# zju3dv/clean-pvnet

Hardware: NVIDIA B200
Metric: ransac_vote_throughput (higher is better)
Workload: dtype f32

## Files before the change

clean_pvnet_b200/csrc/api.cu:

```cuda
#include <cmath>
#include <cstdarg>
#include <cstdio>
#include <cstring>
#include <new>
#include <vector>
#include "kernels.h"

using namespace pvb;

namespace {

thread_local char g_err[512] = "";

int fail(int code, const char *fmt, ...)
{
    va_list ap;
    va_start(ap, fmt);
    vsnprintf(g_err, sizeof(g_err), fmt, ap);
    va_end(ap);
    return code;
}

int cuda_fail(cudaError_t e, const char *what)
{
// ... 55 lines not shown
    if ((long long)d->K * ((d->hn + 511) / 512) > 65535) return fail(PVB_ERR_INVALID, "K*ceil(hn/512) must be <= 65535");
    if (d->mask_dtype < PVB_MASK_U8 || d->mask_dtype > PVB_MASK_F64) return fail(PVB_ERR_INVALID, "bad mask_dtype %d", d->mask_dtype);
    if (d->select_mode != PVB_SELECT_BYTE && d->select_mode != PVB_SELECT_EQ1)
        return fail(PVB_ERR_INVALID, "bad select_mode %d", d->select_mode);
    return PVB_OK;
}

int make_layout(const pvb_desc *d, pvb_layout *L)
{
    const int rc = check_desc(d);
    if (rc) return rc;
    const size_t B = (size_t)d->B, K = (size_t)d->K, hn = (size_t)d->hn;
    const int nwords = (int)(((long long)d->H * d->W + 31) / 32);
    const int nblocks = (nwords + 127) / 128;
    const int cap = default_capacity(d);
    const int splits = refit_splits_for(cap);
    size_t off = 0;
    auto take = [&](size_t bytes) { const size_t o = off; off = align_up(off + bytes); return o; };
    L->status = take(4 * sizeof(int));
    L->fgsum = take(B * sizeof(unsigned long long));
    L->nz = take(B * sizeof(int));
    L->tn = take(B * sizeof(int));
    L->state = take(B * sizeof(int));
    L->refit_ticket = take(B * K * sizeof(int));
    L->ticket = take(B * sizeof(int));
    L->blocktot = take(B * nblocks * sizeof(int));
    L->bits = take(B * nwords * sizeof(uint32_t));
    L->xy = take(B * cap * sizeof(float2));
    L->dirs = take(B * K * cap * sizeof(float2));
    L->hyp = take(B * K * hn * sizeof(float2));
    L->counts = take(B * K * hn * sizeof(int));
    L->win = take(B * K * sizeof(float2));
    L->refit_partial = take(B * K * splits * 5 * sizeof(double));
    L->total = off;
    L->nwords = nwords;
    L->nblocks = nblocks;
    L->capacity = cap;
    L->refit_splits = splits;
    return PVB_OK;
}

struct Plan {
    pvb_layout L;
    SelectArgs s;
    VoteArgs v;
    float2 *win;
    RefitScratch refit;
};

int make_plan(const pvb_desc *d, const void *mask, const float *vertex, const int32_t *idxs,
              const float *selection, void *ws, size_t ws_bytes, uint32_t tag_idx, uint32_t tag_sel, Plan *P)
{
    int rc = make_layout(d, &P->L);
    if (rc) return rc;
    if (!mask || !vertex) return fail(PVB_ERR_INVALID, "mask/vertex is NULL");
    if (!ws || ws_bytes < P->L.total) return fail(PVB_ERR_WORKSPACE, "workspace too small: need %zu bytes, got %zu", P->L.total, ws_bytes);
    if (reinterpret_cast<uintptr_t>(ws) & 255u) return fail(PVB_ERR_WORKSPACE, "workspace must be 256-byte aligned");
    char *w = static_cast<char *>(ws);
    const pvb_layout &L = P->L;
    SelectArgs &s = P->s;
    s.mask = mask; s.mask_dtype = d->mask_dtype; s.select_mode = d->select_mode;
    s.msb = d->mask_stride[0]; s.msy = d->mask_stride[1]; s.msx = d->mask_stride[2];
    s.vertex = vertex;
    for (int i = 0; i < 5; ++i) s.vs[i] = d->vertex_stride[i];
    s.selection = selection;
    s.B = d->B; s.H = d->H; s.W = d->W; s.K = d->K; s.nwords = L.nwords; s.nblocks = L.nblocks; s.cap = L.capacity;
    s.min_num = d->min_num; s.max_num = d->max_num; s.img_base = d->img_base;
    s.seed = d->seed; s.tag_sel = d->rng_tag_sel ? (uint32_t)d->rng_tag_sel : tag_sel;
    s.rowwise_gather = 0;
    s.seg_classes = 0; s.seg_cs = 0; s.mask_out = nullptr;
    s.bits = reinterpret_cast<uint32_t *>(w + L.bits);
    s.blocktot = reinterpret_cast<unsigned *>(w + L.blocktot);
    s.ticket = reinterpret_cast<int *>(w + L.ticket);
    s.fgsum = reinterpret_cast<unsigned long long *>(w + L.fgsum);
    s.nz = reinterpret_cast<int *>(w + L.nz);
    s.tn = reinterpret_cast<int *>(w + L.tn);
    s.state = reinterpret_cast<int *>(w + L.state);
    s.status = reinterpret_cast<int *>(w + L.status);
    s.xy = reinterpret_cast<float2 *>(w + L.xy);
    s.dirs = reinterpret_cast<float2 *>(w + L.dirs);
    VoteArgs &v = P->v;
    v.B = d->B; v.K = d->K; v.hn = d->hn; v.cap = L.capacity; v.W = d->W; v.H = d->H;
    v.thresh = d->inlier_thresh;
    v.tn = s.tn; v.state = s.state; v.xy = s.xy;
    v.dirs = s.dirs; v.idxs = idxs; v.seed = d->seed;
    v.tag_idx = d->rng_tag_idx ? (uint32_t)d->rng_tag_idx : tag_idx;
    v.img_base = d->img_base;
    v.hyp = reinterpret_cast<float2 *>(w + L.hyp);
    v.counts = reinterpret_cast<int *>(w + L.counts);
    P->win = reinterpret_cast<float2 *>(w + L.win);
    P->refit.partial = reinterpret_cast<double *>(w + L.refit_partial);
    P->refit.ticket = reinterpret_cast<int *>(w + L.refit_ticket);
    P->refit.splits = L.refit_splits;
    return PVB_OK;
}

int run_select(const Plan &P, cudaStream_t st)
{
    cudaError_t e = cudaMemsetAsync(P.s.status, 0, P.L.bits, st);
    if (e != cudaSuccess) return cuda_fail(e, "memset(header)");
    e = launch_select(P.s, st);
    if (e != cudaSuccess) return cuda_fail(e, "select kernels");
    return PVB_OK;
}

int run_front(const Plan &P, cudaStream_t st, ProfCall *pc)
{
    prof_start(pc, PVB_STAGE_SELECT, st);
    int rc = run_select(P, st);
    if (rc) return rc;
    prof_end(pc, PVB_STAGE_SELECT, st);
    prof_start(pc, PVB_STAGE_GENERATE, st);
    cudaError_t e = launch_generate(P.v, st);
    if (e != cudaSuccess) return cuda_fail(e, "generate kernel");
    prof_end(pc, PVB_STAGE_GENERATE, st);
    prof_start(pc, PVB_STAGE_VOTE, st);
    e = launch_vote(P.v, false, st);
    if (e != cudaSuccess) return cuda_fail(e, "vote kernel");
    prof_end(pc, PVB_STAGE_VOTE, st);
    return PVB_OK;
}

// ... 393 lines not shown
        di.B = c;
        di.img_base = d->img_base + b0;
        di.capacity = Lc.capacity;
        Plan P;
        rc = make_plan(&di, mptr, vptr, nullptr, nullptr, sb + S.ws, S.end - S.ws, 1u, 2u, &P);
        if (rc) return rc;
        P.s.rowwise_gather = stage_vertex ? 0 : 1;
        rc = run_select(P, hp->in);
        if (rc) return rc;
        e = cudaEventRecord(hp->sel[slot], hp->in);
        if (e == cudaSuccess) e = cudaStreamWaitEvent(hp->cmp, hp->sel[slot], 0);
        if (e != cudaSuccess) return cuda_fail(e, "pipeline event");
        PeerPush none;
        memset(&none, 0, sizeof(none));
        e = launch_generate(P.v, hp->cmp);
        if (e == cudaSuccess) e = launch_vote(P.v, false, hp->cmp);
        if (e == cudaSuccess) e = launch_refit(P.v, P.win, P.refit, reinterpret_cast<float *>(sb + S.out), none, hp->cmp);
        if (e != cudaSuccess) return cuda_fail(e, "compute kernels");
        e = cudaMemcpyAsync(reinterpret_cast<char *>(out_kpt_host) + (size_t)b0 * obytes, sb + S.out, (size_t)c * obytes, cudaMemcpyDeviceToHost, hp->cmp);
        if (e == cudaSuccess) e = cudaEventRecord(hp->done[slot], hp->cmp);
        if (e != cudaSuccess) return cuda_fail(e, "D2H copy");
    }
    e = cudaEventRecord(hp->end, hp->cmp);
    if (e == cudaSuccess) e = cudaStreamWaitEvent(user, hp->end, 0);
    if (e == cudaSuccess) e = cudaStreamSynchronize(user);
    if (e != cudaSuccess) return cuda_fail(e, "stream sync");
    return PVB_OK;
}

PVB_API int pvb_profile_enable(int32_t every) { g_prof_every = every < 0 ? 0 : every; g_prof_tick = 0; return PVB_OK; }

PVB_API int pvb_set_tuning(int32_t gather_mode, int32_t vote_variant)
{
    if (vote_variant < 0 || vote_variant > 3) return fail(PVB_ERR_INVALID, "vote_variant must be 0..3");
    if (gather_mode < 0 || gather_mode > 2) return fail(PVB_ERR_INVALID, "gather_mode must be 0..2");
    set_gather_tuning(gather_mode);
    set_vote_tuning(vote_variant);
    return PVB_OK;
}

PVB_API int pvb_profile_reset(void)
{
    for (auto &pc : g_prof_calls)
        for (auto e : pc.ev) g_prof_pool.push_back(e);
    g_prof_calls.clear();
    return PVB_OK;
}

PVB_API int pvb_profile_read(double *ms, int32_t n)
{
    if (!ms || n < PVB_STAGE_COUNT) return fail(PVB_ERR_INVALID, "ms must hold PVB_STAGE_COUNT doubles");
    int calls = 0;
    for (auto &pc : g_prof_calls) {
        for (int i = 0; i < PVB_STAGE_COUNT; ++i) {
            cudaError_t e = cudaEventSynchronize(pc.ev[i + 1]);
            float t = 0.f;
            if (e == cudaSuccess) e = cudaEventElapsedTime(&t, pc.ev[i], pc.ev[i + 1]);
            if (e != cudaSuccess) { cuda_fail(e, "profile elapsed"); return -1; }
            ms[i] += (double)t;
        }
        if (pc.head) ++calls;
    }
    pvb_profile_reset();
    return calls;
}

static int check_compat(const void *a, const void *b, const void *c, const void *d_, int tn, int vn, int hn)
// ... 22 lines not shown
    cudaError_t e = launch_compat_generate(direct, coords, idxs, hyp, tn, vn, hn, true, static_cast<cudaStream_t>(stream));
    return e == cudaSuccess ? PVB_OK : cuda_fail(e, "generate_hypothesis_vanishing_point");
}

PVB_API int pvb_voting_for_hypothesis(const float *direct, const float *coords, const float *hyp, uint8_t *inliers, int32_t tn,
                              int32_t vn, int32_t hn, float inlier_thresh, pvb_stream_t stream)
{
    int rc = check_compat(direct, coords, hyp, inliers, tn, vn, hn);
    if (rc) return rc;
    if (tn && vn && hn && !inliers) return fail(PVB_ERR_INVALID, "NULL tensor");
    cudaError_t e = launch_compat_vote(direct, coords, hyp, inliers, tn, vn, hn, inlier_thresh, false, static_cast<cudaStream_t>(stream));
    return e == cudaSuccess ? PVB_OK : cuda_fail(e, "voting_for_hypothesis");
}

PVB_API int pvb_voting_for_hypothesis_vanishing_point(const float *direct, const float *coords, const float *hyp,
                                              uint8_t *inliers, int32_t tn, int32_t vn, int32_t hn,
                                              float inlier_thresh, pvb_stream_t stream)
{
    int rc = check_compat(direct, coords, hyp, inliers, tn, vn, hn);
    if (rc) return rc;
    if (tn && vn && hn && !inliers) return fail(PVB_ERR_INVALID, "NULL tensor");
    cudaError_t e = launch_compat_vote(direct, coords, hyp, inliers, tn, vn, hn, inlier_thresh, true, static_cast<cudaStream_t>(stream));
    return e == cudaSuccess ? PVB_OK : cuda_fail(e, "voting_for_hypothesis_vanishing_point");
}

PVB_API size_t pvb_vote_count_workspace_bytes(int32_t tn, int32_t vn, int32_t hn)
{
    if (tn < 0 || vn < 0 || hn < 0) return 0;
    size_t off = align_up(4 * sizeof(int));
    off += align_up((size_t)tn * sizeof(float2));
    off += align_up((size_t)tn * vn * sizeof(float2));
    off += align_up((size_t)hn * vn * sizeof(float2));
    off += align_up((size_t)hn * vn * sizeof(int));
    return off;
}

PVB_API int pvb_vote_count(const float *direct, const float *coords, const float *hyp, int32_t *counts, int32_t tn, int32_t vn,
                   int32_t hn, float inlier_thresh, void *workspace, size_t workspace_bytes, pvb_stream_t stream)
{
    int rc = check_compat(direct, coords, hyp, counts, tn, vn, hn);
    if (rc) return rc;
    cudaStream_t st = static_cast<cudaStream_t>(stream);
    if (hn == 0 || vn == 0) return PVB_OK;
    if (tn == 0) {
        cudaError_t e = cudaMemsetAsync(counts, 0, sizeof(int) * (size_t)hn * vn, st);
        return e == cudaSuccess ? PVB_OK : cuda_fail(e, "memset");
    }
    if ((long long)vn * ((hn + 511) / 512) > 65535) return fail(PVB_ERR_INVALID, "vn*ceil(hn/512) must be <= 65535");
    const size_t need = pvb_vote_count_workspace_bytes(tn, vn, hn);
    if (!workspace || workspace_bytes < need) return fail(PVB_ERR_WORKSPACE, "workspace too small: need %zu", need);
    if (reinterpret_cast<uintptr_t>(workspace) & 255u) return fail(PVB_ERR_WORKSPACE, "workspace must be 256-byte aligned");
    char *w = static_cast<char *>(workspace);
    size_t off = 0;
    int *meta = reinterpret_cast<int *>(w + off); off += align_up(4 * sizeof(int));
    float2 *xy = reinterpret_cast<float2 *>(w + off); off += align_up((size_t)tn * sizeof(float2));
    float2 *dirs = reinterpret_cast<float2 *>(w + off); off += align_up((size_t)tn * vn * sizeof(float2));
    float2 *hyp_k = reinterpret_cast<float2 *>(w + off); off += align_up((size_t)hn * vn * sizeof(float2));
    int *counts_k = reinterpret_cast<int *>(w + off);
    cudaError_t e = launch_compat_repack(direct, coords, hyp, tn, vn, hn, dirs, xy, hyp_k, meta, st);
    if (e != cudaSuccess) return cuda_fail(e, "repack");
    VoteArgs v;
    memset(&v, 0, sizeof(v));
    v.B = 1; v.K = vn; v.hn = hn; v.cap = tn; v.W = 0; v.H = 0; v.thresh = inlier_thresh;
    v.tn = meta; v.state = meta + 1; v.xy = xy;
    v.dirs = dirs; v.idxs = nullptr; v.hyp = hyp_k; v.counts = counts_k;
    e = launch_vote(v, true, st);
    if (e != cudaSuccess) return cuda_fail(e, "vote kernel");
    e = launch_compat_unpack_counts(counts_k, counts, vn, hn, st);
    return e == cudaSuccess ? PVB_OK : cuda_fail(e, "unpack");
}

PVB_API int pvb_exchange_create(int32_t rank, int32_t world, int32_t slots, size_t bytes_per_rank, pvb_exchange **out)
{
    if (!out) return fail(PVB_ERR_INVALID, "out is NULL");
    *out = nullptr;
    if (world < 1 || world > PVB_MAX_PEERS || rank < 0 || rank >= world) return fail(PVB_ERR_INVALID, "bad rank %d / world %d (max %d)", rank, world, PVB_MAX_PEERS);
    if (slots < 2 || slots > 4096) return fail(PVB_ERR_INVALID, "slots must be in [2,4096]");
    if (bytes_per_rank == 0 || bytes_per_rank > ((size_t)1 << 30)) return fail(PVB_ERR_INVALID, "bad bytes_per_rank");
    pvb_exchange *ex = new (std::nothrow) pvb_exchange();
    if (!ex) return fail(PVB_ERR_INVALID, "out of host memory");
    memset(ex, 0, sizeof(*ex));
    ex->rank = rank; ex->world = world; ex->slots = slots;
    ex->bytes_per_rank = (bytes_per_rank + 15) / 16 * 16;
    ex->status_off = align_up((size_t)slots * world * ex->bytes_per_rank * 2);
    ex->total = ex->status_off + 256;
    cudaError_t e = cudaGetDevice(&ex->device);
    if (e == cudaSuccess) e = cudaMalloc(reinterpret_cast<void **>(&ex->local), ex->total);
    if (e == cudaSuccess) e = cudaMemset(ex->local, 0, ex->total);
    if (e == cudaSuccess) e = cudaDeviceSynchronize();
    if (e != cudaSuccess) { if (ex->local) cudaFree(ex->local); delete ex; return cuda_fail(e, "exchange allocation"); }
    ex->peer[rank] = ex->local;
    ex->connected = (world == 1);
    *out = ex;
    return PVB_OK;
}

PVB_API size_t pvb_exchange_bytes_per_rank(const pvb_exchange *ex) { return ex ? ex->bytes_per_rank : 0; }
PVB_API void *pvb_exchange_base(const pvb_exchange *ex) { return ex ? ex->local : nullptr; }
// ... 90 lines not shown
```

clean_pvnet_b200/csrc/common.cuh:

```cuda
#pragma once
#include <cuda_runtime.h>
#include <stdint.h>

namespace pvb {

__device__ __forceinline__ uint4 philox4x32_10(uint4 c, uint2 k)
{
#pragma unroll
    for (int r = 0; r < 10; ++r) {
        const uint32_t hi0 = __umulhi(0xD2511F53u, c.x), lo0 = 0xD2511F53u * c.x;
        const uint32_t hi1 = __umulhi(0xCD9E8D57u, c.z), lo1 = 0xCD9E8D57u * c.z;
        c = make_uint4(hi1 ^ c.y ^ k.x, lo1, hi0 ^ c.w ^ k.y, lo0);
        k.x += 0x9E3779B9u;
        k.y += 0xBB67AE85u;
    }
    return c;
}

__device__ __forceinline__ float u32_to_unit(uint32_t x) { return (float)(x >> 8) * 5.9604644775390625e-08f; }

__device__ __forceinline__ bool hypothesis_from_pair(float dx0, float dy0, float cx0, float cy0,
                                                     float dx1, float dy1, float cx1, float cy1,
                                                     float &x, float &y)
{
// ... 29 lines not shown
{
#pragma unroll
    for (int o = 16; o > 0; o >>= 1) v += __shfl_xor_sync(0xffffffffu, v, o);
    return v;
}
__device__ __forceinline__ double warp_sum(double v)
{
#pragma unroll
    for (int o = 16; o > 0; o >>= 1) v += __shfl_xor_sync(0xffffffffu, v, o);
    return v;
}
__device__ __forceinline__ int warp_sum(int v) { return __reduce_add_sync(0xffffffffu, v); }

__device__ __forceinline__ void cov_to_weights(const float4 c, float &o0, float &o1, float &o2)
{
    o0 = 0.f; o1 = 0.f; o2 = 0.f;
    const bool bad = (c.x < 1e-6f) || (c.x != c.x) || (c.y != c.y) || (c.z != c.z) || (c.w != c.w);
    if (!bad) {
        const double a = c.x, b = 0.5 * ((double)c.y + (double)c.z), d = c.w;
        const double det = a * d - b * b;
        if (det > 0.0) {
            const double s = sqrt(det), t = sqrt(a + d + 2.0 * s);
            const double a2 = a + s, d2 = d + s;
            const double den = a2 * d2 - b * b;
            o0 = (float)(t * d2 / den); o1 = (float)(-t * b / den); o2 = (float)(t * a2 / den);
        }
    }
}

struct ConeParams {
    float kappa;
    float band;
    float thresh;
};

}
```

clean_pvnet_b200/csrc/kernels.h:

```cpp
#pragma once
#include <cuda_runtime.h>
#include <stdint.h>
#include "../../include/pvnet_vote_b200.h"

namespace pvb {

struct SelectArgs {
    const void *mask;
    int mask_dtype, select_mode;
    long long msb, msy, msx;
    const float *vertex;
    long long vs[5];
    const float *selection;
    int B, H, W, K, nwords, nblocks, cap, min_num, max_num, img_base;
    int rowwise_gather;
    int seg_classes;
    long long seg_cs;
    long long *mask_out;
    uint64_t seed;
    uint32_t tag_sel;
    uint32_t *bits;
    unsigned *blocktot;
    int *ticket;
    unsigned long long *fgsum;
    int *nz, *tn, *state, *status;
    float2 *xy, *dirs;
};
cudaError_t launch_select(const SelectArgs &a, cudaStream_t st);

struct VoteArgs {
    int B, K, hn, cap, W, H;
    float thresh;
    const int *tn;
    const int *state;
    const float2 *xy;
    const float2 *dirs;
    const int32_t *idxs;
    uint64_t seed;
    uint32_t tag_idx;
    int img_base;
    float2 *hyp;
    int *counts;
};
cudaError_t launch_generate(const VoteArgs &a, cudaStream_t st);
cudaError_t launch_vote(const VoteArgs &a, bool zero_counts, cudaStream_t st);
void set_vote_tuning(int variant);
void set_gather_tuning(int mode);
struct RefitScratch { double *partial; int *ticket; int splits; };
int refit_splits_for(int cap);
constexpr int PVB_MAX_PEERS = 16;
struct PeerPush {
    int world;
    unsigned int seq;
    uint2 *recv[PVB_MAX_PEERS];
};
cudaError_t launch_refit(const VoteArgs &a, float2 *win, const RefitScratch &rs, float *out_kpt, const PeerPush &pp,
                         cudaStream_t st);
struct ExchangeCounts { int n[PVB_MAX_PEERS]; };
cudaError_t launch_exchange_wait(const uint2 *recv, unsigned int seq, float *out, int world, int stride_words,
                                 const ExchangeCounts &counts, unsigned long long timeout_ns, int *status, cudaStream_t st);
cudaError_t launch_covariance(const VoteArgs &a, const float *mean, float *out_cov, const PeerPush &pp, cudaStream_t st);

cudaError_t launch_pnp_weights(const float *cov, float *w, int n, cudaStream_t st);

struct PnpArgs {
    const double *pts2d;
    const double *pts3d;
    const double *wgt2d;
    const double *K;
    const double *init_rt;
    double *result_rt;
    int *info;
    int n, pn;
    long long pts3d_stride, k_stride;
    int max_num_iterations;
    double function_tolerance, gradient_tolerance, parameter_tolerance;
};
cudaError_t launch_pnp(const PnpArgs &a, cudaStream_t st);
cudaError_t launch_p3p_init(const PnpArgs &a, cudaStream_t st);
// ... 30 lines not shown
```

clean_pvnet_b200/csrc/vote.cu:

```cuda
#include <atomic>
#include <math_constants.h>
#include "common.cuh"
#include "kernels.h"

namespace pvb {

__global__ void __launch_bounds__(256)
generate_kernel(VoteArgs a)
{
    const int h = blockIdx.x * 256 + threadIdx.x;
    if (h >= a.hn) return;
    const int k = blockIdx.y, b = blockIdx.z;
    const int tn = min(a.tn[b], a.cap);
    float x = 0.f, y = 0.f;
    if (tn > 0) {
        int t0, t1;
        if (a.idxs) {
            const int2 t = __ldg(reinterpret_cast<const int2 *>(a.idxs) + ((size_t)b * a.hn + h) * a.K + k);
            t0 = t.x; t1 = t.y;
        } else {
            const uint4 r = philox4x32_10(make_uint4((uint32_t)h, (uint32_t)k, (uint32_t)(a.img_base + b), a.tag_idx),
                                          make_uint2((uint32_t)a.seed, (uint32_t)(a.seed >> 32)));
            t0 = (int)(r.x % (uint32_t)tn);
            t1 = (int)(r.y % (uint32_t)tn);
        }
        if ((unsigned)t0 < (unsigned)tn && (unsigned)t1 < (unsigned)tn) {
            const float2 *dk = a.dirs + ((size_t)b * a.K + k) * a.cap;
            const float2 *xy = a.xy + (size_t)b * a.cap;
            const float2 d0 = dk[t0], d1 = dk[t1], c0 = xy[t0], c1 = xy[t1];
            float hx, hy;
            if (hypothesis_from_pair(d0.x, d0.y, c0.x, c0.y, d1.x, d1.y, c1.x, c1.y, hx, hy)) { x = hx; y = hy; }
        }
    }
    a.hyp[((size_t)b * a.K + k) * a.hn + h] = make_float2(x, y);
    a.counts[((size_t)b * a.K + k) * a.hn + h] = 0;
}

cudaError_t launch_generate(const VoteArgs &a, cudaStream_t st)
{
    dim3 g((a.hn + 255) / 256, a.K, a.B);
    generate_kernel<<<g, 256, 0, st>>>(a);
    return cudaGetLastError();
}

struct VoteK {
    VoteArgs a;
    ConeParams cone;
};

constexpr int VOTE_BLOCK = 16;

__device__ __forceinline__ float4 lds128(uint32_t addr)
{
    float4 v;
    asm volatile("ld.shared.v4.f32 {%0,%1,%2,%3}, [%4];" : "=f"(v.x), "=f"(v.y), "=f"(v.z), "=f"(v.w) : "r"(addr) : "memory");
    return v;
}

__device__ __forceinline__ float cone_margin(const float4 ra, const float2 rb, float hxc, float hyc)
{
    const float ap = fmaf(ra.x, hxc, fmaf(ra.y, hyc, ra.z));
    const float pp = fmaf(ra.w, hxc, fmaf(rb.x, hyc, rb.y));
    return ap - fabsf(pp);
}

template <int HPT, int NT, int MINB, int VOTE_TILE, int WS>
__global__ void __launch_bounds__(NT, MINB)
vote_kernel(const VoteK p)
{
    constexpr int PPT = VOTE_TILE / NT;
    constexpr int NW = NT / 32;
    constexpr int TEAM = WS * 32;
    constexpr int TEAMS = NT / TEAM;
    __shared__ __align__(16) float4 s_a[VOTE_TILE];
    __shared__ __align__(16) float2 s_b[VOTE_TILE];
    __shared__ float s_box[4][NW];
    const VoteArgs &a = p.a;
    const int b = blockIdx.z;
    const int k = blockIdx.y % a.K, slice = blockIdx.y / a.K;
    const int tn = min(a.tn[b], a.cap);
    const int t0 = blockIdx.x * VOTE_TILE;
    if (t0 >= tn) return;
    const int n = min(VOTE_TILE, tn - t0);
    const int npad = (n + VOTE_BLOCK - 1) / VOTE_BLOCK * VOTE_BLOCK;
    const int tid = threadIdx.x, lane = tid & 31, warp = tid >> 5;
    const float kappa = p.cone.kappa, thresh = p.cone.thresh;
    const float2 *hyp = a.hyp + ((size_t)b * a.K + k) * a.hn;
    const float2 *xy = a.xy + (size_t)b * a.cap + t0;
    const float2 *dk = a.dirs + ((size_t)b * a.K + k) * a.cap + t0;
    const int team = tid / TEAM;
    const int hbase = slice * (TEAM * HPT) + (tid - team * TEAM);

    float2 v[PPT], c[PPT];
    float x0 = CUDART_INF_F, x1 = -CUDART_INF_F, y0 = CUDART_INF_F, y1 = -CUDART_INF_F;
#pragma unroll
    for (int r = 0; r < PPT; ++r) {
        const int i = tid + r * NT;
        v[r] = make_float2(0.f, 0.f); c[r] = make_float2(0.f, 0.f);
        if (i < n) {
            v[r] = __ldg(dk + i); c[r] = __ldg(xy + i);
            x0 = fminf(x0, c[r].x); x1 = fmaxf(x1, c[r].x); y0 = fminf(y0, c[r].y); y1 = fmaxf(y1, c[r].y);
        }
// ... 87 lines not shown
#pragma unroll
            for (int j = 0; j < HPT; ++j) {
                unsigned bm = __ballot_sync(0xffffffffu, mn[j] < dl[j]);
                while (bm) {
                    const int L = __ffs(bm) - 1;
                    bm &= bm - 1;
                    const float hx_ = __shfl_sync(0xffffffffu, hxc[j], L), hy_ = __shfl_sync(0xffffffffu, hyc[j], L);
                    const float dl_ = __shfl_sync(0xffffffffu, dl[j], L);
                    const int h = hbase - lane + L + j * TEAM;
                    const float2 q = (h < a.hn) ? __ldg(hyp + h) : make_float2(0.f, 0.f);
                    int delta = 0;
                    if (lane < nb) {
                        const float m = cone_margin(ra, rb, hx_, hy_);
                        if (fabsf(m) < dl_) {
                            const bool in = vote_exact(vv.x, vv.y, cc.x, cc.y, q.x, q.y, thresh);
                            delta = (in ? 0 : 1) - (int)(__float_as_uint(m) >> 31);
                        }
                    }
                    delta = __reduce_add_sync(0xffffffffu, delta);
                    if (lane == L) neg[j] += delta;
                }
            }
        }
    }
    int *counts = a.counts + ((size_t)b * a.K + k) * a.hn;
#pragma unroll
    for (int j = 0; j < HPT; ++j) {
        const int h = hbase + j * TEAM;
        const int cnt = mine - neg[j];
        if (h < a.hn && cnt) atomicAdd(counts + h, cnt);
    }
}

ConeParams make_cone(float thresh)
{
    ConeParams c;
    c.thresh = thresh;
    const double t = (double)thresh;
    if (t > 0.0 && t < 1.0) {
        const double s = sqrt(1.0 - t * t);
        const double kappa = s / t, G = 1.0 / (t * s);
        const double band = 1.25 * ldexp(1.0, -24) * (18.0 + 22.0 * kappa + 9.0 * G);
        c.kappa = (float)kappa;
        c.band = nextafterf((float)band, INFINITY);
    } else {
        c.kappa = 0.f;
        c.band = INFINITY;
    }
    return c;
}

static std::atomic<int> g_vote_variant{0};

void set_vote_tuning(int variant) { g_vote_variant.store(variant, std::memory_order_relaxed); }

cudaError_t launch_vote(const VoteArgs &a, bool zero_counts, cudaStream_t st)
{
    if (zero_counts) {
        cudaError_t e = cudaMemsetAsync(a.counts, 0, sizeof(int) * (size_t)a.B * a.K * a.hn, st);
        if (e != cudaSuccess) return e;
    }
    VoteK p;
    p.a = a;
    p.cone = make_cone(a.thresh);
    const int variant = g_vote_variant.load(std::memory_order_relaxed);
#define PVB_VOTE(HPT, NT, MINB, TILE, WS)                                               \
    do {                                                                                \
        const int slices = (a.hn + (HPT) * (WS) * 32 - 1) / ((HPT) * (WS) * 32);        \
        dim3 g((a.cap + (TILE) - 1) / (TILE), a.K * slices, a.B);                       \
        vote_kernel<HPT, NT, MINB, TILE, WS><<<g, NT, 0, st>>>(p);                      \
    } while (0)
    if (a.hn <= 32) PVB_VOTE(1, 128, 8, 512, 1);
    else if (a.hn <= 64) PVB_VOTE(2, 128, 8, 512, 1);
    else if (a.hn <= 128) PVB_VOTE(4, 128, 8, 512, 1);
    else if (a.hn <= 256) PVB_VOTE(4, 128, 8, 512, 2);
    else if (variant == 2) PVB_VOTE(4, 128, 8, 256, 4);
    else if (variant == 3) PVB_VOTE(4, 128, 8, 1024, 4);
    else PVB_VOTE(4, 128, 8, 512, 4);
#undef PVB_VOTE
    return cudaGetLastError();
}

template <int NV>
__device__ __forceinline__ void peer_push(const PeerPush &pp, size_t bk, const float (&v)[NV])
{
    for (int r = 0; r < pp.world; ++r) {
        uint2 *dst = pp.recv[r] + bk * NV;
#pragma unroll
        for (int i = 0; i < NV; ++i)
            asm volatile("st.volatile.global.v2.u32 [%0], {%1, %2};" ::"l"(dst + i), "r"(__float_as_uint(v[i])), "r"(pp.seq) : "memory");
    }
}

constexpr int RF_THREADS = 128;
constexpr int RF_CHUNK = 2048;

int refit_splits_for(int cap) { return (cap + RF_CHUNK - 1) / RF_CHUNK; }

__device__ __forceinline__ bool vote_winner(float vx, float vy, float cx, float cy, float hx, float hy,
                                            const ConeParams &cone)
{
    const float dx = __fsub_rn(hx, cx), dy = __fsub_rn(hy, cy);
    const float n1sq = fmaf(vx, vx, vy * vy);
    const float S = fabsf(dx) + fabsf(dy);
    const float m = cone.kappa * fmaf(vx, dx, vy * dy) - fabsf(fmaf(vx, dy, -(vy * dx)));
    const float thr = cone.band * S;
    const bool safe = (n1sq > 1e-10f) && (n1sq < 1e8f) && (S <= 1e6f) && (m * m > thr * thr * n1sq * 1.0001f);
    return safe ? (m > 0.f) : vote_exact(vx, vy, cx, cy, hx, hy, cone.thresh);
}

__global__ void __launch_bounds__(RF_THREADS)
refit_kernel(VoteArgs a, float2 *__restrict__ win, RefitScratch rs, float *__restrict__ out, ConeParams cone, PeerPush pp)
{
    const int split = blockIdx.x, k = blockIdx.y, b = blockIdx.z;
    const int tid = threadIdx.x, lane = tid & 31, warp = tid >> 5;
    constexpr int NW = RF_THREADS / 32;
    const int tn = min(a.tn[b], a.cap);
    const size_t bk = (size_t)b * a.K + k;
    __shared__ int s_c[NW], s_h[NW];
    __shared__ double s_acc[NW][5];
    __shared__ int s_last;
    float2 res = make_float2(0.f, 0.f);
    if (a.state[b] != 0 || tn <= 0) {
        if (split != 0) return;
        if (tid == 0) { out[bk * 2] = 0.f; out[bk * 2 + 1] = 0.f; win[bk] = make_float2(0.f, 0.f); }
    } else {
        const int nsplit = (tn + RF_CHUNK - 1) / RF_CHUNK;
        if (split >= nsplit) return;
        const int *counts = a.counts + bk * a.hn;
        int bc = -1, bh = 0x7fffffff;
        for (int h = tid; h < a.hn; h += RF_THREADS) {
            const int c = counts[h];
            if (c > bc) { bc = c; bh = h; }
        }
#pragma unroll
        for (int o = 16; o > 0; o >>= 1) {
            const int oc = __shfl_xor_sync(0xffffffffu, bc, o), oh = __shfl_xor_sync(0xffffffffu, bh, o);
            if (oc > bc || (oc == bc && oh < bh)) { bc = oc; bh = oh; }
        }
        if (lane == 0) { s_c[warp] = bc; s_h[warp] = bh; }
        __syncthreads();
#pragma unroll
        for (int w = 0; w < NW; ++w)
            if (s_c[w] > bc || (s_c[w] == bc && s_h[w] < bh)) { bc = s_c[w]; bh = s_h[w]; }
        const float2 wpt = (bc > 0) ? a.hyp[bk * a.hn + bh] : make_float2(0.f, 0.f);
        if (split == 0 && tid == 0) win[bk] = wpt;
// ... 28 lines not shown
            double *pq = rs.partial + (bk * rs.splits + split) * 5;
            for (int i = 0; i < 5; ++i) {
                double s = 0;
                for (int w = 0; w < NW; ++w) s += s_acc[w][i];
                __stcg(pq + i, s);
            }
            __threadfence();
            s_last = (atomicAdd(rs.ticket + bk, 1) == nsplit - 1);
        }
        __syncthreads();
        if (!s_last) return;
        if (tid == 0) {
            __threadfence();
            double s[5] = {0, 0, 0, 0, 0};
            for (int sp = 0; sp < nsplit; ++sp)
                for (int i = 0; i < 5; ++i) s[i] += __ldcg(rs.partial + (bk * rs.splits + sp) * 5 + i);
            const double det = s[0] * s[2] - s[1] * s[1];
            float x, y;
            if (det == 0.0 || !isfinite(det)) { x = (float)s[3]; y = (float)s[4]; }
            else { x = (float)((s[2] * s[3] - s[1] * s[4]) / det); y = (float)((s[0] * s[4] - s[1] * s[3]) / det); }
            out[bk * 2] = x; out[bk * 2 + 1] = y;
            res = make_float2(x, y);
        }
    }
    if (pp.world <= 0 || tid != 0) return;
    const float v[2] = {res.x, res.y};
    peer_push<2>(pp, bk, v);
}

cudaError_t launch_refit(const VoteArgs &a, float2 *win, const RefitScratch &rs, float *out_kpt, const PeerPush &pp,
                         cudaStream_t st)
{
    dim3 g(rs.splits, a.K, a.B);
    refit_kernel<<<g, RF_THREADS, 0, st>>>(a, win, rs, out_kpt, make_cone(a.thresh), pp);
    return cudaGetLastError();
}

constexpr int CV_THREADS = 256;

__global__ void __launch_bounds__(CV_THREADS)
covariance_kernel(VoteArgs a, const float *__restrict__ mean, float *__restrict__ cov, PeerPush pp)
{
    const int k = blockIdx.x, b = blockIdx.y;
    const int tid = threadIdx.x, lane = tid & 31, warp = tid >> 5;
    const size_t bk = (size_t)b * a.K + k;
    const int tn = min(a.tn[b], a.cap);
    const bool skipped = a.state[b] != 0;
    const int *counts = a.counts + bk * a.hn;
    const float2 *hyp = a.hyp + bk * a.hn;
    const float ftn = (float)tn;
    __shared__ float s_max[CV_THREADS / 32];
    __shared__ double s_acc[CV_THREADS / 32][4];
    float mx = -CUDART_INF_F;
    bool has_nan = false;
    for (int h = tid; h < a.hn; h += CV_THREADS) {
        const float r = skipped ? 1.f : __fdiv_rn((float)counts[h], ftn);
        if (r != r) has_nan = true;
        mx = fmaxf(mx, r);
    }
#pragma unroll
    for (int o = 16; o > 0; o >>= 1) mx = fmaxf(mx, __shfl_xor_sync(0xffffffffu, mx, o));
    if (lane == 0) s_max[warp] = mx;
    __syncthreads();
    mx = s_max[0];
    for (int w = 1; w < CV_THREADS / 32; ++w) mx = fmaxf(mx, s_max[w]);
    (void)has_nan;
    const float th = __fsub_rn(mx, 0.1f);
    const float mx_ = mean[bk * 2], my_ = mean[bk * 2 + 1];
// ... 49 lines not shown
```

Baseline: 224,700.

## Add PDL launches and opt-in Morton-sorted culled vote kernel variant

Launches the generate, vote and refit kernels with programmatic dependent launch, and adds griddepcontrol.wait at kernel entry, so launch latency can overlap the tail of the previous kernel. It also adds vote variant 4: hypotheses are sorted by Morton code per keypoint, then a culling kernel bounds each cluster of four hypotheses with a Lipschitz cone test and only falls back to the exact per-hypothesis vote near the boundary. The sorted path is opt-in and needs extra workspace for the permutation. PDL applies by default and risks ordering subtleties if any kernel reads producer data before its wait.

```diff
diff --git a/clean_pvnet_b200/csrc/api.cu b/clean_pvnet_b200/csrc/api.cu
--- a/clean_pvnet_b200/csrc/api.cu
+++ b/clean_pvnet_b200/csrc/api.cu
@@ -111,6 +111,7 @@
     L->counts = take(B * K * hn * sizeof(int));
     L->win = take(B * K * sizeof(float2));
     L->refit_partial = take(B * K * splits * 5 * sizeof(double));
+    take(B * K * hn * sizeof(int));
     L->total = off;
     L->nwords = nwords;
     L->nblocks = nblocks;
@@ -167,6 +168,8 @@
     v.img_base = d->img_base;
     v.hyp = reinterpret_cast<float2 *>(w + L.hyp);
     v.counts = reinterpret_cast<int *>(w + L.counts);
+    v.perm = vote_uses_perm(d->hn) ? reinterpret_cast<int *>(w + L.total - align_up((size_t)d->B * d->K * d->hn * sizeof(int)))
+                                   : nullptr;
     P->win = reinterpret_cast<float2 *>(w + L.win);
     P->refit.partial = reinterpret_cast<double *>(w + L.refit_partial);
     P->refit.ticket = reinterpret_cast<int *>(w + L.refit_ticket);
@@ -626,7 +629,7 @@
 
 PVB_API int pvb_set_tuning(int32_t gather_mode, int32_t vote_variant)
 {
-    if (vote_variant < 0 || vote_variant > 3) return fail(PVB_ERR_INVALID, "vote_variant must be 0..3");
+    if (vote_variant < 0 || vote_variant > 4) return fail(PVB_ERR_INVALID, "vote_variant must be 0..4");
     if (gather_mode < 0 || gather_mode > 2) return fail(PVB_ERR_INVALID, "gather_mode must be 0..2");
     set_gather_tuning(gather_mode);
     set_vote_tuning(vote_variant);
@@ -715,6 +718,7 @@
     off += align_up((size_t)tn * vn * sizeof(float2));
     off += align_up((size_t)hn * vn * sizeof(float2));
     off += align_up((size_t)hn * vn * sizeof(int));
+    off += align_up((size_t)hn * vn * sizeof(int));
     return off;
 }
 
@@ -739,7 +743,8 @@
     float2 *xy = reinterpret_cast<float2 *>(w + off); off += align_up((size_t)tn * sizeof(float2));
     float2 *dirs = reinterpret_cast<float2 *>(w + off); off += align_up((size_t)tn * vn * sizeof(float2));
     float2 *hyp_k = reinterpret_cast<float2 *>(w + off); off += align_up((size_t)hn * vn * sizeof(float2));
-    int *counts_k = reinterpret_cast<int *>(w + off);
+    int *counts_k = reinterpret_cast<int *>(w + off); off += align_up((size_t)hn * vn * sizeof(int));
+    int *perm = reinterpret_cast<int *>(w + off);
     cudaError_t e = launch_compat_repack(direct, coords, hyp, tn, vn, hn, dirs, xy, hyp_k, meta, st);
     if (e != cudaSuccess) return cuda_fail(e, "repack");
     VoteArgs v;
@@ -747,6 +752,7 @@
     v.B = 1; v.K = vn; v.hn = hn; v.cap = tn; v.W = 0; v.H = 0; v.thresh = inlier_thresh;
     v.tn = meta; v.state = meta + 1; v.xy = xy;
     v.dirs = dirs; v.idxs = nullptr; v.hyp = hyp_k; v.counts = counts_k;
+    v.perm = vote_uses_perm(hn) ? perm : nullptr;
     e = launch_vote(v, true, st);
     if (e != cudaSuccess) return cuda_fail(e, "vote kernel");
     e = launch_compat_unpack_counts(counts_k, counts, vn, hn, st);
diff --git a/clean_pvnet_b200/csrc/common.cuh b/clean_pvnet_b200/csrc/common.cuh
--- a/clean_pvnet_b200/csrc/common.cuh
+++ b/clean_pvnet_b200/csrc/common.cuh
@@ -85,6 +85,7 @@
     float kappa;
     float band;
     float thresh;
+    float lip;
 };
 
 }
diff --git a/clean_pvnet_b200/csrc/kernels.h b/clean_pvnet_b200/csrc/kernels.h
--- a/clean_pvnet_b200/csrc/kernels.h
+++ b/clean_pvnet_b200/csrc/kernels.h
@@ -41,10 +41,12 @@
     int img_base;
     float2 *hyp;
     int *counts;
+    int *perm;
 };
 cudaError_t launch_generate(const VoteArgs &a, cudaStream_t st);
 cudaError_t launch_vote(const VoteArgs &a, bool zero_counts, cudaStream_t st);
 void set_vote_tuning(int variant);
+bool vote_uses_perm(int hn);
 void set_gather_tuning(int mode);
 struct RefitScratch { double *partial; int *ticket; int splits; };
 int refit_splits_for(int cap);
diff --git a/clean_pvnet_b200/csrc/vote.cu b/clean_pvnet_b200/csrc/vote.cu
--- a/clean_pvnet_b200/csrc/vote.cu
+++ b/clean_pvnet_b200/csrc/vote.cu
@@ -1,17 +1,27 @@
 #include <atomic>
+#include <utility>
 #include <math_constants.h>
 #include "common.cuh"
 #include "kernels.h"
 
 namespace pvb {
 
-__global__ void __launch_bounds__(256)
-generate_kernel(VoteArgs a)
-{
-    const int h = blockIdx.x * 256 + threadIdx.x;
-    if (h >= a.hn) return;
-    const int k = blockIdx.y, b = blockIdx.z;
-    const int tn = min(a.tn[b], a.cap);
+__device__ __forceinline__ void pdl_wait() { asm volatile("griddepcontrol.wait;" ::: "memory"); }
+
+template <typename... P, typename... A>
+static cudaError_t launch_pdl(void (*kernel)(P...), dim3 grid, dim3 block, size_t smem, cudaStream_t st, A &&...args)
+{
+    cudaLaunchConfig_t cfg = {};
+    cfg.gridDim = grid; cfg.blockDim = block; cfg.dynamicSmemBytes = smem; cfg.stream = st;
+    cudaLaunchAttribute attr[1];
+    attr[0].id = cudaLaunchAttributeProgrammaticStreamSerialization;
+    attr[0].val.programmaticStreamSerializationAllowed = 1;
+    cfg.attrs = attr; cfg.numAttrs = 1;
+    return cudaLaunchKernelEx(&cfg, kernel, std::forward<A>(args)...);
+}
+
+__device__ __forceinline__ float2 make_hypothesis(const VoteArgs &a, int b, int k, int h, int tn)
+{
     float x = 0.f, y = 0.f;
     if (tn > 0) {
         int t0, t1;
@@ -32,15 +42,74 @@
             if (hypothesis_from_pair(d0.x, d0.y, c0.x, c0.y, d1.x, d1.y, c1.x, c1.y, hx, hy)) { x = hx; y = hy; }
         }
     }
-    a.hyp[((size_t)b * a.K + k) * a.hn + h] = make_float2(x, y);
+    return make_float2(x, y);
+}
+
+__global__ void __launch_bounds__(256)
+generate_kernel(VoteArgs a)
+{
+    pdl_wait();
+    const int h = blockIdx.x * 256 + threadIdx.x;
+    if (h >= a.hn) return;
+    const int k = blockIdx.y, b = blockIdx.z;
+    a.hyp[((size_t)b * a.K + k) * a.hn + h] = make_hypothesis(a, b, k, h, min(a.tn[b], a.cap));
     a.counts[((size_t)b * a.K + k) * a.hn + h] = 0;
 }
 
+__global__ void __launch_bounds__(1024)
+generate_sorted_kernel(VoteArgs a, int gen)
+{
+    extern __shared__ unsigned long long s_key[];
+    const int k = blockIdx.x, b = blockIdx.y, tid = threadIdx.x, nts = blockDim.x;
+    const size_t bk = (size_t)b * a.K + k;
+    unsigned long long key = ~0ull;
+    if (tid < a.hn) {
+        float2 q;
+        if (gen) {
+            q = make_hypothesis(a, b, k, tid, min(a.tn[b], a.cap));
+            a.hyp[bk * a.hn + tid] = q;
+            a.counts[bk * a.hn + tid] = 0;
+        } else {
+            q = a.hyp[bk * a.hn + tid];
+        }
+        uint32_t code = 0xffffffffu;
+        if (isfinite(q.x) && isfinite(q.y)) {
+            const uint32_t qx = (uint32_t)fminf(fmaxf(q.x * 8.f + 32768.f, 0.f), 65535.f);
+            const uint32_t qy = (uint32_t)fminf(fmaxf(q.y * 8.f + 32768.f, 0.f), 65535.f);
+            code = 0;
+#pragma unroll
+            for (int i = 0; i < 16; ++i) code |= (((qx >> i) & 1u) << (2 * i)) | (((qy >> i) & 1u) << (2 * i + 1));
+        }
+        key = ((unsigned long long)code << 32) | (uint32_t)tid;
+    }
+    s_key[tid] = key;
+    __syncthreads();
+    for (int len = 2; len <= nts; len <<= 1) {
+        for (int j = len >> 1; j > 0; j >>= 1) {
+            const int o = tid ^ j;
+            if (o > tid) {
+                const unsigned long long x = s_key[tid], y = s_key[o];
+                if ((x > y) == ((tid & len) == 0)) { s_key[tid] = y; s_key[o] = x; }
+            }
+            __syncthreads();
+        }
+    }
+    if (tid < a.hn) a.perm[bk * a.hn + tid] = (int)(uint32_t)s_key[tid];
+}
+
+static cudaError_t launch_generate_sorted(const VoteArgs &a, bool gen, cudaStream_t st)
+{
+    int nts = 32;
+    while (nts < a.hn) nts <<= 1;
+    generate_sorted_kernel<<<dim3(a.K, a.B), nts, nts * sizeof(unsigned long long), st>>>(a, gen ? 1 : 0);
+    return cudaGetLastError();
+}
+
 cudaError_t launch_generate(const VoteArgs &a, cudaStream_t st)
 {
+    if (a.perm) return launch_generate_sorted(a, true, st);
     dim3 g((a.hn + 255) / 256, a.K, a.B);
-    generate_kernel<<<g, 256, 0, st>>>(a);
-    return cudaGetLastError();
+    return launch_pdl(generate_kernel, g, dim3(256), 0, st, a);
 }
 
 struct VoteK {
@@ -68,6 +137,7 @@
 __global__ void __launch_bounds__(NT, MINB)
 vote_kernel(const VoteK p)
 {
+    pdl_wait();
     constexpr int PPT = VOTE_TILE / NT;
     constexpr int NW = NT / 32;
     constexpr int TEAM = WS * 32;
@@ -221,6 +291,204 @@
     }
 }
 
+constexpr int CULL_NT = 128;
+constexpr int CULL_TILE = 512;
+constexpr int CULL_CL = 4;
+constexpr int CULL_SLICE = CULL_NT * CULL_CL;
+
+__global__ void __launch_bounds__(CULL_NT, 8)
+vote_cull_kernel(const VoteK p)
+{
+    constexpr int CL = CULL_CL, NT = CULL_NT, VOTE_TILE = CULL_TILE;
+    constexpr int PPT = VOTE_TILE / NT;
+    constexpr int NW = NT / 32;
+    __shared__ __align__(16) float4 s_a[VOTE_TILE];
+    __shared__ __align__(16) float2 s_b[VOTE_TILE];
+    __shared__ __align__(16) float4 s_hx[NT], s_hy[NT], s_dl[NT];
+    __shared__ unsigned s_cnt[NT];
+    __shared__ unsigned s_und[NW][32];
+    __shared__ float s_box[4][NW];
+    const VoteArgs &a = p.a;
+    const int b = blockIdx.z;
+    const int k = blockIdx.y % a.K, slice = blockIdx.y / a.K;
+    const int tn = min(a.tn[b], a.cap);
+    const int t0 = blockIdx.x * VOTE_TILE;
+    if (t0 >= tn) return;
+    const int n = min(VOTE_TILE, tn - t0);
+    const int npad = (n + 31) & ~31;
+    const int tid = threadIdx.x, lane = tid & 31, warp = tid >> 5;
+    const float kappa = p.cone.kappa, thresh = p.cone.thresh;
+    const size_t bk = (size_t)b * a.K + k;
+    const float2 *hyp = a.hyp + bk * a.hn;
+    const int *perm = a.perm + bk * a.hn;
+    const float2 *xy = a.xy + (size_t)b * a.cap + t0;
+    const float2 *dk = a.dirs + bk * a.cap + t0;
+
+    float2 v[PPT], c[PPT];
+    float x0 = CUDART_INF_F, x1 = -CUDART_INF_F, y0 = CUDART_INF_F, y1 = -CUDART_INF_F;
+#pragma unroll
+    for (int r = 0; r < PPT; ++r) {
+        const int i = tid + r * NT;
+        v[r] = make_float2(0.f, 0.f); c[r] = make_float2(0.f, 0.f);
+        if (i < n) {
+            v[r] = __ldg(dk + i); c[r] = __ldg(xy + i);
+            x0 = fminf(x0, c[r].x); x1 = fmaxf(x1, c[r].x); y0 = fminf(y0, c[r].y); y1 = fmaxf(y1, c[r].y);
+        }
+    }
+#pragma unroll
+    for (int o = 16; o > 0; o >>= 1) {
+        x0 = fminf(x0, __shfl_xor_sync(0xffffffffu, x0, o)); x1 = fmaxf(x1, __shfl_xor_sync(0xffffffffu, x1, o));
+        y0 = fminf(y0, __shfl_xor_sync(0xffffffffu, y0, o)); y1 = fmaxf(y1, __shfl_xor_sync(0xffffffffu, y1, o));
+    }
+    if (lane == 0) { s_box[0][warp] = x0; s_box[1][warp] = x1; s_box[2][warp] = y0; s_box[3][warp] = y1; }
+    __syncthreads();
+#pragma unroll
+    for (int w = 0; w < NW; ++w) {
+        x0 = fminf(x0, s_box[0][w]); x1 = fmaxf(x1, s_box[1][w]); y0 = fminf(y0, s_box[2][w]); y1 = fmaxf(y1, s_box[3][w]);
+    }
+    const float ox = 0.5f * (x0 + x1), oy = 0.5f * (y0 + y1);
+    const float cmax = (0.5f * (x1 - x0) + 0.5f * (y1 - y0)) * 1.000001f + 1e-3f;
+#pragma unroll
+    for (int r = 0; r < PPT; ++r) {
+        const int i = tid + r * NT;
+        if (i < npad) {
+            float4 ra = make_float4(0.f, 0.f, -1e30f, 0.f);
+            float2 rb = make_float2(0.f, 0.f);
+            if (i < n) {
+                const float n1 = __fsqrt_rn(__fmaf_rn(v[r].x, v[r].x, __fmul_rn(v[r].y, v[r].y)));
+                const float cxc = c[r].x - ox, cyc = c[r].y - oy;
+                if (!(n1 > below_1e6())) {
+                } else if (!(n1 < 1e18f) || !(fabsf(cxc) + fabsf(cyc) <= cmax)) {
+                    ra.z = 0.f;
+                } else {
+                    const float inv = 1.0f / n1;
+                    const float ux = v[r].x * inv, uy = v[r].y * inv;
+                    const float a1 = kappa * ux, a2 = kappa * uy;
+                    ra.x = a1; ra.y = a2; ra.z = -fmaf(a1, cxc, a2 * cyc);
+                    ra.w = -uy; rb.x = ux; rb.y = fmaf(uy, cxc, -(ux * cyc));
+                }
+            }
+            s_a[i] = ra; s_b[i] = rb;
+        }
+    }
+
+    const int s0 = CL * (slice * NT + tid);
+    float hx[CL], hy[CL], dl[CL];
+    bool any_exact = false;
+    int present = 0;
+    float bx0 = CUDART_INF_F, bx1 = -CUDART_INF_F, by0 = CUDART_INF_F, by1 = -CUDART_INF_F;
+#pragma unroll
+    for (int j = 0; j < CL; ++j) {
+        hx[j] = 0.f; hy[j] = 0.f; dl[j] = 0.f;
+        if (s0 + j < a.hn) {
+            ++present;
+            const float2 q = hyp[perm[s0 + j]];
+            float xc = q.x - ox, yc = q.y - oy;
+            const float S = fabsf(xc) + fabsf(yc) + cmax;
+            float d = fmaxf(p.cone.band * S, 1e-30f);
+            if (!(S <= 1e15f) || !(d < CUDART_INF_F)) { xc = 0.f; yc = 0.f; d = CUDART_INF_F; any_exact = true; }
+            else { bx0 = fminf(bx0, xc); bx1 = fmaxf(bx1, xc); by0 = fminf(by0, yc); by1 = fmaxf(by1, yc); }
+            hx[j] = xc; hy[j] = yc; dl[j] = d;
+        }
+    }
+    float Hx = 0.f, Hy = 0.f, thr;
+    if (present == 0) {
+        thr = -CUDART_INF_F;
+    } else if (any_exact) {
+        thr = CUDART_INF_F;
+    } else {
+        Hx = 0.5f * (bx0 + bx1); Hy = 0.5f * (by0 + by1);
+        float r = 0.f;
+#pragma unroll
+        for (int j = 0; j < CL; ++j)
+            if (s0 + j < a.hn) {
+                const float dx = hx[j] - Hx, dy = hy[j] - Hy;
+                r = fmaxf(r, sqrtf(dx * dx + dy * dy));
+            }
+        const float Scl = fabsf(Hx) + fabsf(Hy) + 1.41422f * r + cmax;
+        thr = (p.cone.lip * r + p.cone.band * Scl) * 1.000001f;
+        if (!(thr < CUDART_INF_F)) { thr = CUDART_INF_F; Hx = 0.f; Hy = 0.f; }
+    }
+    s_hx[tid] = make_float4(hx[0], hx[1], hx[2], hx[3]);
+    s_hy[tid] = make_float4(hy[0], hy[1], hy[2], hy[3]);
+    s_dl[tid] = make_float4(dl[0], dl[1], dl[2], dl[3]);
+    s_cnt[tid] = 0u;
+    __syncthreads();
+
+    const uint32_t sa0 = (uint32_t)__cvta_generic_to_shared(s_a);
+    const uint32_t sb0 = (uint32_t)__cvta_generic_to_shared(s_b);
+    int cin = 0;
+    int cnt[CL];
+#pragma unroll
+    for (int j = 0; j < CL; ++j) cnt[j] = 0;
+    unsigned *und = s_und[warp];
+    const int cw = warp * 32;
+    for (int i0 = 0; i0 < npad; i0 += 32) {
+        const uint32_t sa = sa0 + (uint32_t)i0 * 16u, sb = sb0 + (uint32_t)i0 * 8u;
+#pragma unroll
+        for (int u = 0; u < 32; u += 2) {
+            const float4 ra0 = lds128(sa + u * 16), ra1 = lds128(sa + u * 16 + 16);
+            const float4 rbb = lds128(sb + u * 8);
+            const float m0 = cone_margin(ra0, make_float2(rbb.x, rbb.y), Hx, Hy);
+            const float m1 = cone_margin(ra1, make_float2(rbb.z, rbb.w), Hx, Hy);
+            cin += (int)(__float_as_uint(thr - m0) >> 31);
+            cin += (int)(__float_as_uint(thr - m1) >> 31);
+            const unsigned b0 = __ballot_sync(0xffffffffu, !(fabsf(m0) > thr));
+            const unsigned b1 = __ballot_sync(0xffffffffu, !(fabsf(m1) > thr));
+            if (lane == 0) { und[u] = b0; und[u + 1] = b1; }
+        }
+        __syncwarp();
+        unsigned todo = (i0 + lane < n) ? und[lane] : 0u;
+        if (__any_sync(0xffffffffu, todo != 0u)) {
+            const float4 ra = s_a[i0 + lane];
+            const float2 rb = s_b[i0 + lane];
+            while (todo) {
+                const int L = __ffs(todo) - 1;
+                todo &= todo - 1;
+                const float4 qx = s_hx[cw + L], qy = s_hy[cw + L], qd = s_dl[cw + L];
+                const float qxa[4] = {qx.x, qx.y, qx.z, qx.w}, qya[4] = {qy.x, qy.y, qy.z, qy.w};
+                const float qda[4] = {qd.x, qd.y, qd.z, qd.w};
+                unsigned inc = 0u;
+                bool near = false;
+#pragma unroll
+                for (int j = 0; j < CL; ++j) {
+                    const float m = cone_margin(ra, rb, qxa[j], qya[j]);
+                    inc |= (unsigned)(m > 0.f) << (8 * j);
+                    near |= fabsf(m) < qda[j];
+                }
+                if (near) {
+                    const float2 vv = __ldg(dk + i0 + lane), cc = __ldg(xy + i0 + lane);
+                    const int sc = CL * (slice * NT + cw + L);
+#pragma unroll
+                    for (int j = 0; j < CL; ++j) {
+                        const float m = cone_margin(ra, rb, qxa[j], qya[j]);
+                        if (fabsf(m) < qda[j]) {
+                            const float2 q = __ldg(hyp + perm[sc + j]);
+                            const bool in = vote_exact(vv.x, vv.y, cc.x, cc.y, q.x, q.y, thresh);
+                            inc = (inc & ~(0xffu << (8 * j))) | ((unsigned)in << (8 * j));
+                        }
+                    }
+                }
+                if (inc) atomicAdd(&s_cnt[cw + L], inc);
+            }
+        }
+        __syncwarp();
+        const unsigned w = s_cnt[tid];
+        if (w) {
+#pragma unroll
+            for (int j = 0; j < CL; ++j) cnt[j] += (int)((w >> (8 * j)) & 0xffu);
+            s_cnt[tid] = 0u;
+        }
+        __syncwarp();
+    }
+    int *counts = a.counts + bk * a.hn;
+#pragma unroll
+    for (int j = 0; j < CL; ++j) {
+        const int cc = cin + cnt[j];
+        if (s0 + j < a.hn && cc) atomicAdd(counts + perm[s0 + j], cc);
+    }
+}
+
 ConeParams make_cone(float thresh)
 {
     ConeParams c;
@@ -232,9 +500,11 @@
         const double band = 1.25 * ldexp(1.0, -24) * (18.0 + 22.0 * kappa + 9.0 * G);
         c.kappa = (float)kappa;
         c.band = nextafterf((float)band, INFINITY);
+        c.lip = nextafterf((float)sqrt(1.0 + kappa * kappa), INFINITY);
     } else {
         c.kappa = 0.f;
         c.band = INFINITY;
+        c.lip = INFINITY;
     }
     return c;
 }
@@ -242,6 +512,12 @@
 static std::atomic<int> g_vote_variant{0};
 
 void set_vote_tuning(int variant) { g_vote_variant.store(variant, std::memory_order_relaxed); }
+
+bool vote_uses_perm(int hn)
+{
+    const int variant = g_vote_variant.load(std::memory_order_relaxed);
+    return variant == 4 && hn > 256 && hn <= 1024;
+}
 
 cudaError_t launch_vote(const VoteArgs &a, bool zero_counts, cudaStream_t st)
 {
@@ -252,12 +528,23 @@
     VoteK p;
     p.a = a;
     p.cone = make_cone(a.thresh);
+    if (a.perm) {
+        if (zero_counts) {
+            cudaError_t e = launch_generate_sorted(a, false, st);
+            if (e != cudaSuccess) return e;
+        }
+        const int slices = (a.hn + CULL_SLICE - 1) / CULL_SLICE;
+        dim3 g((a.cap + CULL_TILE - 1) / CULL_TILE, a.K * slices, a.B);
+        vote_cull_kernel<<<g, CULL_NT, 0, st>>>(p);
+        return cudaGetLastError();
+    }
     const int variant = g_vote_variant.load(std::memory_order_relaxed);
+    cudaError_t e = cudaSuccess;
 #define PVB_VOTE(HPT, NT, MINB, TILE, WS)                                               \
     do {                                                                                \
         const int slices = (a.hn + (HPT) * (WS) * 32 - 1) / ((HPT) * (WS) * 32);        \
         dim3 g((a.cap + (TILE) - 1) / (TILE), a.K * slices, a.B);                       \
-        vote_kernel<HPT, NT, MINB, TILE, WS><<<g, NT, 0, st>>>(p);                      \
+        e = launch_pdl(vote_kernel<HPT, NT, MINB, TILE, WS>, g, dim3(NT), 0, st, p);    \
     } while (0)
     if (a.hn <= 32) PVB_VOTE(1, 128, 8, 512, 1);
     else if (a.hn <= 64) PVB_VOTE(2, 128, 8, 512, 1);
@@ -267,7 +554,7 @@
     else if (variant == 3) PVB_VOTE(4, 128, 8, 1024, 4);
     else PVB_VOTE(4, 128, 8, 512, 4);
 #undef PVB_VOTE
-    return cudaGetLastError();
+    return e;
 }
 
 template <int NV>
@@ -301,6 +588,7 @@
 __global__ void __launch_bounds__(RF_THREADS)
 refit_kernel(VoteArgs a, float2 *__restrict__ win, RefitScratch rs, float *__restrict__ out, ConeParams cone, PeerPush pp)
 {
+    pdl_wait();
     const int split = blockIdx.x, k = blockIdx.y, b = blockIdx.z;
     const int tid = threadIdx.x, lane = tid & 31, warp = tid >> 5;
     constexpr int NW = RF_THREADS / 32;
@@ -395,8 +683,7 @@
                          cudaStream_t st)
 {
     dim3 g(rs.splits, a.K, a.B);
-    refit_kernel<<<g, RF_THREADS, 0, st>>>(a, win, rs, out_kpt, make_cone(a.thresh), pp);
-    return cudaGetLastError();
+    return launch_pdl(refit_kernel, g, dim3(RF_THREADS), 0, st, a, win, rs, out_kpt, make_cone(a.thresh), pp);
 }
 
 constexpr int CV_THREADS = 256;
```

After: 226,300, median of 6. About the same (+0.7%).
